# ahmetaa/fast-dnn

Measured on AMD Instinct MI355X. Metric: acoustic frames/sec (whole node), 7x2048->8000 nnet, higher is better.
Workload: dtype int8 (u8 activations x s8 weights -> int32; fp32 layer 0 and soft-max)

## Files before the change

fast-dnn_amd/api.py:

```python
from __future__ import annotations

import ctypes as C
import os
import subprocess
from typing import Optional, Sequence

import numpy as np

_HERE = os.path.dirname(os.path.abspath(__file__))
LIB_PATH = os.environ.get("FDNN_LIB") or os.path.join(_HERE, "lib", "libfast-dnn.so")
CSRC = os.path.join(_HERE, "csrc")

FDNN_OK, FDNN_E_ARG, FDNN_E_IO, FDNN_E_FORMAT, FDNN_E_DEVICE, FDNN_E_NOMEM, FDNN_E_STATE = 0, -1, -2, -3, -4, -5, -6


class FdnnError(RuntimeError):
    def __init__(self, code: int, msg: str):
        super().__init__(f"fdnn error {code}: {msg}")
        self.code = code


def build(verbose: bool = False) -> str:
    jobs = str(max(1, min(8, os.cpu_count() or 1)))
    subprocess.check_call(["make", "-C", CSRC, "-j", jobs, "all"] + ([] if verbose else ["-s"]))
# ... 23 lines not shown
    "fdnn_model_set_l0_fma": (C.c_int, [C.c_void_p, C.c_int]),
    "fdnn_debug_set_l0_kernel": (C.c_int, [C.c_void_p, C.c_int]),
    "fdnn_debug_set_chain": (C.c_int, [C.c_int, C.c_int]),
    "fdnn_model_chain_faults": (C.c_int, [C.c_void_p, C.POINTER(C.c_ulonglong)]),
    "fdnn_debug_set_pp": (C.c_int, [C.c_int, C.c_int]),
    "fdnn_debug_set_ppo": (C.c_int, [C.c_int]),
    "fdnn_debug_launch_name_count": (C.c_int, []),
    "fdnn_debug_launch_name": (C.c_char_p, [C.c_int, C.POINTER(C.c_int)]),
    "fdnn_debug_launch_record": (C.c_int, [C.c_int]),
    "fdnn_debug_launch_reset": (C.c_int, []),
    "fdnn_debug_launch_counts": (C.c_int, [C.POINTER(C.c_ulonglong), C.c_int]),
    "fdnn_debug_raise_fuse_fault": (C.c_int, [C.c_void_p, C.c_int]),
    "fdnn_device_shared": (C.c_int, [C.c_int]),
    "fdnn_debug_set_fuse": (C.c_int, [C.c_int]),
    "fdnn_debug_set_l0_list_cap": (C.c_int, [C.c_void_p, C.c_int]),
    "fdnn_debug_chain_clocks": (C.c_int, [C.c_void_p, C.POINTER(C.c_longlong), C.c_int]),
    "fdnn_calculate": (C.c_int, [C.c_void_p, _c_f32p, C.c_int, C.c_int, C.c_int, _c_f32p]),
    "fdnn_calculate_device": (C.c_int, [C.c_void_p, C.c_void_p, C.c_int, C.c_void_p, C.c_void_p]),
    "fdnn_calculate_lazy": (C.c_int, [C.c_void_p, _c_f32p, C.c_int, C.c_int, _c_i8p, _c_f32p]),
    "fdnn_calculate_lazy_bits": (C.c_int, [C.c_void_p, _c_f32p, C.c_int, C.c_int, C.POINTER(C.c_uint64), _c_f32p]),
    "fdnn_calculate_lazy_bits_device": (C.c_int, [C.c_void_p, C.c_void_p, C.c_int, C.c_void_p, C.c_void_p, C.c_void_p]),
    "fdnn_ctx_create": (C.c_int, [C.c_void_p, C.c_int, C.c_int, C.POINTER(C.c_void_p)]),
    "fdnn_ctx_free": (None, [C.c_void_p]),
    "fdnn_ctx_frame_count": (C.c_int, [C.c_void_p]),
    "fdnn_ctx_output_dim": (C.c_int, [C.c_void_p]),
    "fdnn_ctx_forward_hidden": (C.c_int, [C.c_void_p, _c_f32p]),
    "fdnn_ctx_forward_hidden_device": (C.c_int, [C.c_void_p, C.c_void_p, C.c_void_p]),
    "fdnn_ctx_lazy_output": (C.c_int, [C.c_void_p, C.c_int, _c_i8p, _c_f32p]),
    "fdnn_ctx_lazy_output_batch": (C.c_int, [C.c_void_p, C.c_int, C.c_int, _c_i8p, _c_f32p]),
    "fdnn_ctx_lazy_output_batch_device": (C.c_int, [C.c_void_p, C.c_int, C.c_int, C.c_void_p, C.c_void_p, C.c_void_p]),
# ... 123 lines not shown
def device_count() -> int:
    return int(lib().fdnn_device_count())


def device_shared(device: int = 0) -> bool:
    r = int(lib().fdnn_device_shared(int(device)))
    if r < 0:
        _check(r)
    return r == 1


def set_fuse(mode: int) -> None:
    _check(lib().fdnn_debug_set_fuse(int(mode)))


def set_chain(mode: int, min_frames: int = 0) -> None:
    _check(lib().fdnn_debug_set_chain(int(mode), int(min_frames)))


def set_pp(mode: int, min_frames: int = 0) -> None:
    _check(lib().fdnn_debug_set_pp(int(mode), int(min_frames)))


def set_ppo(mode: int) -> None:
    _check(lib().fdnn_debug_set_ppo(int(mode)))


LAUNCH_ABLATION, LAUNCH_LOAD_TIME = 1, 2


# ... 621 lines not shown
```

fast-dnn_amd/csrc/fdnn_debug.cpp:

```cpp
#include <hip/hip_runtime.h>

#include <algorithm>
#include <atomic>
#include <cstring>
#include <mutex>
#include <string>
#include <vector>

#include "fdnn_internal.hpp"

using namespace fdnn;

struct fdnn_host_model {
  fdnn::HostModel hm;
};

namespace fdnn {
const LaunchNameInfo kLaunchNames[kLaunchNameCount] = {
#define FDNN_X(id, name, flags) {name, flags},
    FDNN_LAUNCH_NAMES(FDNN_X)
#undef FDNN_X
#define FDNN_G(out, shape, branch, name, abl) {name, abl},
        FDNN_GEMM_LAUNCH_NAMES(FDNN_G)
#undef FDNN_G
// ... 40 lines not shown
    fdnn::lazy_expand_rows_from(out, comp, count, size_t(O), size_t(stride), bits);
  }
  lazy_expand_force_scalar(false);
  return FDNN_OK;
}

int fdnn_debug_set_l0_list_cap(fdnn_model *m, int cap) {
  if (!m || cap < 0) return fail(FDNN_E_ARG, "bad argument");
  std::lock_guard<std::mutex> lk(m->mu);
  for (fdnn_ctx *c : m->pool) destroy_ctx(c);
  m->pool.clear();
  m->l0_list_cap = cap;
  return FDNN_OK;
}

int fdnn_debug_set_pp(int mode, int min_frames) {
  if (mode < -1 || mode > 1) return fail(FDNN_E_ARG, "pp mode must be -1, 0 or 1");
  fdnn::qpp_set_mode(mode, min_frames);
  return FDNN_OK;
}

int fdnn_debug_raise_fuse_fault(fdnn_model *m, int value) {
  if (!m) return fail(FDNN_E_ARG, "null model");
  if (!m->h_fuse_fault) return fail(FDNN_E_STATE, "this model has no fault word");
  __atomic_store_n(m->h_fuse_fault, value ? 1ull : 0ull, __ATOMIC_RELAXED);
  if (!value) m->fuse_fault_said = false;
  return FDNN_OK;
}

int fdnn_debug_set_ppo(int mode) {
// ... 172 lines not shown
  const BlobHeader &h = m->hm.hdr;
  fdnn_ctx *c = nullptr;
  int rc = make_ctx(m, n, &c);
  if (rc) return rc;
  const size_t outs = size_t(n) * h.hidden;
  unsigned long long before[2] = {0, 0}, after[2] = {0, 0};
  hipError_t e = hipSuccess;
  if (screen) {
    e = hipMalloc(reinterpret_cast<void **>(&c->d_l0_dbg_t), outs * sizeof(float));
    if (e == hipSuccess) e = hipMalloc(reinterpret_cast<void **>(&c->d_l0_dbg_dd), outs * sizeof(float));
    if (e == hipSuccess) e = hipMemset(c->d_l0_dbg_t, 0xff, outs * sizeof(float));
    if (e == hipSuccess) e = hipMemset(c->d_l0_dbg_dd, 0xff, outs * sizeof(float));
    if (e == hipSuccess) e = hipDeviceSynchronize();
  }
  if (e == hipSuccess) e = hipMemcpy(before, m->d_l0_stats, sizeof(before), hipMemcpyDeviceToHost);
  if (e == hipSuccess) e = hipMemcpyAsync(c->d_x, x, sizeof(float) * size_t(n) * h.in_dim, hipMemcpyHostToDevice, c->stream);
  if (e == hipSuccess) {
    const int kernel_before = m->l0_kernel;
    if (screen && m->l0_kernel == 0) m->l0_kernel = 4;
    run_layer0(c, c->d_x, c->stream, nullptr);
    m->l0_kernel = kernel_before;
    e = hipGetLastError();
  }
  std::vector<int8_t> tmp(size_t(n) * size_t(c->act_ld));
  if (e == hipSuccess) e = hipMemcpyAsync(tmp.data(), c->d_act[0], tmp.size(), hipMemcpyDeviceToHost, c->stream);
  if (e == hipSuccess && screen) e = hipMemcpyAsync(t_out, c->d_l0_dbg_t, outs * sizeof(float), hipMemcpyDeviceToHost, c->stream);
  if (e == hipSuccess && screen) e = hipMemcpyAsync(dd_out, c->d_l0_dbg_dd, outs * sizeof(float), hipMemcpyDeviceToHost, c->stream);
  if (e == hipSuccess) e = hipStreamSynchronize(c->stream);
  if (e == hipSuccess) e = hipMemcpy(after, m->d_l0_stats, sizeof(after), hipMemcpyDeviceToHost);
  const size_t act_ld = size_t(c->act_ld);
// ... 158 lines not shown
```

fast-dnn_amd/csrc/fdnn_kernels.hpp:

```cpp
#pragma once
#include <hip/hip_runtime.h>

#include <cstdint>
#include <vector>

#include "fdnn_note.hpp"

#ifdef FDNN_ABLATION
#include <cstdlib>
#define FDNN_TUNE_ENV(name) std::getenv(name)
#else
#define FDNN_TUNE_ENV(name) static_cast<const char *>(nullptr)
#if (defined(FDNN_GEMM_DEBUG) && FDNN_GEMM_DEBUG) || (defined(FDNN_L0S_DEBUG) && FDNN_L0S_DEBUG) || (defined(FDNN_L0_DEBUG) && FDNN_L0_DEBUG) || \
    (defined(FDNN_CHAIN_CLK) && FDNN_CHAIN_CLK) || defined(FDNN_L0S_CLK) || defined(FDNN_GEMM_PAD)
#error "ablation / clock builds need -DFDNN_ABLATION (tools/build_variant.sh)"
#endif
#endif

namespace fdnn {

constexpr int kMaxFrameTile = 320;
constexpr int kPartialNodes = 64;

struct L0Params {
// ... 23 lines not shown
  float *xstat;
  const int8_t *wd;
  const float *wstat;
  uint2 *glist;
  uint32_t *glist_count;
  int glist_cap;
  const uint32_t *luthalf;
  float *dbg_t;
  float *dbg_dd;
};
constexpr int kL0ScreenCap = 4096;
void launch_l0(const L0Params &p, hipStream_t s);
bool l0_split_ok(int D, int H);
size_t l0_split_plane_bytes(int D, int rows_ld);
void launch_l0_split(const L0Params &p, hipStream_t s);
void l0_split_build_weights(const float *w, const float *wnorm, const uint8_t *lut2, int H, int D, int h_ld, std::vector<int8_t> *planes,
                            std::vector<float> *stat, std::vector<uint32_t> *half);
int l0_chunk_rows(int D);
int l0_chain_node_tile();
void launch_l0_weight_image(const float *w, float *wt, int H, int D, int j_pad, int h_ld, hipStream_t s);

int qgemm_frame_tile(int rows_pad, int n);
int qgemm_node_tile(int rows_pad, int n, bool output);
int qgemm_debug_flags();

struct QGemmParams {
  const int8_t *w;
  const int8_t *a;
  const float *bias;
  const int32_t *wsum;
// ... 99 lines not shown
```

fast-dnn_amd/csrc/fdnn_l0s.hip:

```cpp
#include <atomic>
#include <cmath>
#include <cstdlib>
#include <limits>
#include <type_traits>
#include <vector>

#include "fdnn_device.hpp"
#include "fdnn_kernels.hpp"

namespace fdnn {

namespace {

#ifndef FDNN_L0S_DEBUG
#define FDNN_L0S_DEBUG 0
#endif
constexpr float kU = 5.9604645e-8f;
constexpr int kSplitW = 32;

[[maybe_unused]] __device__ __forceinline__ bool split_tile_of_block(int node_tiles, int frame_tiles, int &bx, int &by) {
  const int b = blockIdx.x, xcd = b & 7, slot = b >> 3;
  bx = slot % node_tiles;
  by = xcd + 8 * (slot / node_tiles);
  return by < frame_tiles;
}

constexpr int kDigFrames = 8;
__global__ __launch_bounds__(256) void l0_digits_kernel(L0Params p, int KC, int J, int JP) {
  extern __shared__ __attribute__((aligned(16))) float dig_smem[];
  const int D = p.D, ld = D + 1;
  float *xs = dig_smem;
  float *cf_s = dig_smem + kDigFrames * ld;
  const int tid = threadIdx.x, f0 = blockIdx.x * kDigFrames;
  if (blockIdx.x == 0 && tid < 2) p.glist_count[tid] = 0u;
  const int quads = D >> 2;
  {
    float4 raw[4], sh[4], sc[4];
    int rowq[4];
#pragma unroll
    for (int it = 0; it < 4; ++it) {
// ... 91 lines not shown
      char *base = reinterpret_cast<char *>(p.xd) + ((static_cast<size_t>(kc) * 3 + pl) * blocks + (f >> 5)) * 1024 + hh * 512 + (f & 31) * 16;
      *reinterpret_cast<uint4 *>(base) = make_uint4(d[0], d[1], d[2], d[3]);
    }
  }
}

constexpr int kSTF = 128, kSStages = 3;
template <int WN>
struct SplitCfg {
  static constexpr int TN = 64 * WN, NW = 4 * WN, THREADS = 64 * NW;
  static constexpr int PIECES = 12 + 6 * WN;
  static constexpr int STAGE = PIECES * 1024;
  static constexpr int RING = STAGE * kSStages;
  static constexpr int HALF_OFF = RING;
  static constexpr int STAT_OFF = RING + 11 * 1024;
  static constexpr int LDS = STAT_OFF + 3 * 1024;
  static constexpr int TS = TN + 16;
  static constexpr int PPW = (PIECES + NW - 1) / NW;
  static_assert(kSTF * TS + 16 + 2 * kL0ScreenCap <= RING, "epilogue tile and flag list must fit in the dead ring");
};
static_assert(4 * kLut2Size <= 11 * 1024, "half-step table area");

template <int WN, bool DBG = false>
__global__ __launch_bounds__(256 * WN, 3 - WN) void l0_split_kernel(L0Params p, int KC, int CPC) {
#if defined(__HIP_DEVICE_COMPILE__)
  using Cfg = SplitCfg<WN>;
  constexpr int kSTN = Cfg::TN, kSStage = Cfg::STAGE, kSTS = Cfg::TS, kSHalfOff = Cfg::HALF_OFF, kSStatOff = Cfg::STAT_OFF, NW = Cfg::NW;
  extern __shared__ __attribute__((aligned(16))) char smem[];
  const int tid = threadIdx.x, lane = tid & 63;
  const int wave = __builtin_amdgcn_readfirstlane(tid >> 6);
  const int l32 = lane & 31, h = lane >> 5;
  const int wf = wave & 3, wn = wave >> 2;
  const int node_tiles = p.h_ld / kSTN, frame_tiles = (p.n_rows + kSTF - 1) / kSTF;
  int bx, by;
  if (!split_tile_of_block(node_tiles, frame_tiles, bx, by)) return;
  const int f0 = by * kSTF, n0 = bx * kSTN;
  const int xblocks = p.n_ld >> 5, wblocks = p.h_ld >> 5;
#ifdef FDNN_L0S_CLK
  long long tc[12];
  tc[0] = __builtin_readcyclecounter();
#define L0S_TS(i) tc[i] = __builtin_readcyclecounter()
#else
#define L0S_TS(i)
#endif

  {
    const __amdgpu_buffer_rsrc_t rsrc_half =
        __builtin_amdgcn_make_buffer_rsrc(const_cast<uint32_t *>(p.luthalf), 0, (4 * kLut2Size + 15) & ~15, 0x00020000);
#pragma unroll
    for (int i = 0; i < 14; ++i) {
      if (i % NW != wave) continue;
      if (i < 11) {
        __builtin_amdgcn_raw_ptr_buffer_load_lds(rsrc_half, FDNN_LDS_PTR(smem + kSHalfOff + i * 1024), 16, lane * 16, i * 1024, 0, 0);
      } else {
        const int q = i - 11;
        const __amdgpu_buffer_rsrc_t rsrc_st =
            __builtin_amdgcn_make_buffer_rsrc(const_cast<float *>(p.xstat + static_cast<size_t>(q) * p.n_ld + f0), 0, kSTF * 4, 0x00020000);
        __builtin_amdgcn_raw_ptr_buffer_load_lds(rsrc_st, FDNN_LDS_PTR(smem + kSStatOff + q * 1024), 16, lane * 16, 0, 0, 0);
      }
    }
  }
  const __amdgpu_buffer_rsrc_t rsrc_x =
      __builtin_amdgcn_make_buffer_rsrc(const_cast<int8_t *>(p.xd), 0, static_cast<unsigned>(KC) * 3u * static_cast<unsigned>(xblocks) * 1024u, 0x00020000);
  const __amdgpu_buffer_rsrc_t rsrc_w = __builtin_amdgcn_make_buffer_rsrc(
      const_cast<int8_t *>(p.wd), 0, static_cast<unsigned>(KC) * 3u * static_cast<unsigned>(wblocks) * 1024u, 0x00020000);
  const int voff = lane * 16;
  const int my_pieces = (Cfg::PIECES - wave + NW - 1) / NW;
  auto stage_piece = [&](int kc, int buf, int t) {
    char *base = smem + buf * kSStage;
    const int i = wave + NW * t;
    if (i >= Cfg::PIECES) return;
    if (i < 12) {
      const int pl = i >> 2, q = i & 3;
      __builtin_amdgcn_raw_ptr_buffer_load_lds(rsrc_x, FDNN_LDS_PTR(base + i * 1024), 16, voff, ((kc * 3 + pl) * xblocks + (f0 >> 5) + q) * 1024, 0, 0);
    } else {
      const int j = i - 12, pl = j / (2 * WN), q = j % (2 * WN);
      __builtin_amdgcn_raw_ptr_buffer_load_lds(rsrc_w, FDNN_LDS_PTR(base + i * 1024), 16, voff, ((kc * 3 + pl) * wblocks + (n0 >> 5) + q) * 1024, 0, 0);
    }
  };
  auto stage = [&](int kc, int buf) {
#pragma unroll
    for (int t = 0; t < Cfg::PPW; ++t) stage_piece(kc, buf, t);
  };
  auto wait_stages = [&](int stages) {
    if (stages == 0) {
      asm volatile("s_waitcnt vmcnt(0) lgkmcnt(0)" ::: "memory");
    } else if (Cfg::PIECES % NW == 0) {
      if (stages == 1)
        asm volatile("s_waitcnt vmcnt(%0) lgkmcnt(0)" ::"n"(Cfg::PPW) : "memory");
      else
        asm volatile("s_waitcnt vmcnt(%0) lgkmcnt(0)" ::"n"(2 * Cfg::PPW) : "memory");
    } else if (my_pieces == Cfg::PPW) {
      if (stages == 1)
        asm volatile("s_waitcnt vmcnt(%0) lgkmcnt(0)" ::"n"(Cfg::PPW) : "memory");
      else
        asm volatile("s_waitcnt vmcnt(%0) lgkmcnt(0)" ::"n"(2 * Cfg::PPW) : "memory");
    } else {
      if (stages == 1)
        asm volatile("s_waitcnt vmcnt(%0) lgkmcnt(0)" ::"n"(Cfg::PPW - 1) : "memory");
      else
        asm volatile("s_waitcnt vmcnt(%0) lgkmcnt(0)" ::"n"(2 * (Cfg::PPW - 1)) : "memory");
    }
  };
  stage(0, 0);
  stage(1, 1);
  stage(2, 2);
  asm volatile("" ::: "memory");

  constexpr int kP0Off = 0x40000000;
  v16i P0[2], P1[2], P2[2];
  uint32_t A[2][16];
#pragma unroll
  for (int s = 0; s < 2; ++s)
#pragma unroll
    for (int r = 0; r < 16; ++r) {
      P0[s][r] = kP0Off; P1[s][r] = 0; P2[s][r] = 0;
      A[s][r] = 0u;
    }
  auto chain_end = [&](int s) {
#pragma unroll
    for (int r = 0; r < 16; ++r) {
      P1[s][r] += P0[s][r] << 8;
      P0[s][r] = kP0Off;
    }
  };
  v4i xa[2][3], wb[2][3][2];
  auto load_plane = [&](int buf, int set, int pl) {
    const char *sb = smem + buf * kSStage;
    xa[set][pl] = *reinterpret_cast<const v4i *>(sb + (pl * 4 + wf) * 1024 + lane * 16);
#pragma unroll
    for (int s = 0; s < 2; ++s) wb[set][pl][s] = *reinterpret_cast<const v4i *>(sb + 12288 + (pl * 2 * WN + wn * 2 + s) * 1024 + lane * 16);
  };
  auto load_frags = [&](int buf, int set) {
// ... 31 lines not shown
    P1[s] = __builtin_amdgcn_mfma_i32_32x32x32_i8(xa[set][1], wb[set][0][s], P1[s], 0, 0, 0);
    FDNN_L0S_FENCE;
    sample_part(ss, 9, 12, on);
    x3();
    FDNN_L0S_FENCE;
    P2[s] = __builtin_amdgcn_mfma_i32_32x32x32_i8(xa[set][1], wb[set][1][s], P2[s], 0, 0, 0);
    FDNN_L0S_FENCE;
    sample_part(ss, 12, 16, on);
    x4();
    FDNN_L0S_FENCE;
    P2[s] = __builtin_amdgcn_mfma_i32_32x32x32_i8(xa[set][2], wb[set][0][s], P2[s], 0, 0, 0);
    FDNN_L0S_FENCE;
  };
  auto nothing = [] {};

  wait_stages(2);
  __builtin_amdgcn_s_barrier();
  asm volatile("" ::: "memory");
  load_frags(0, 0);
  L0S_TS(1);
  auto chunk = [&](int kc, auto set_c, auto first_c, bool chain_start) {
    constexpr int set = decltype(set_c)::value;
    constexpr bool first = decltype(first_c)::value;
    if (chain_start) chain_end(0);
    mfma_group(set, 0, 1, !first, nothing, nothing, nothing, nothing, nothing);
    const bool more = kc + 1 < KC, refill = kc + 3 < KC && !(FDNN_L0S_DEBUG & 8);
    if (more) {
      wait_stages(kc + 2 < KC ? 1 : 0);
      if (!(FDNN_L0S_DEBUG & 16)) __builtin_amdgcn_s_barrier();
      asm volatile("" ::: "memory");
    }
    if (chain_start) chain_end(1);
    const int nb = (kc + 1) % 3;
    mfma_group(
        set, 1, 0, true, [&] { if (more && !(FDNN_L0S_DEBUG & 32)) load_plane(nb, set ^ 1, 0); if (refill) stage_piece(kc + 3, kc % 3, 0); },
        [&] { if (more && !(FDNN_L0S_DEBUG & 32)) load_plane(nb, set ^ 1, 1); if (refill) stage_piece(kc + 3, kc % 3, 1); },
        [&] { if (more && !(FDNN_L0S_DEBUG & 32)) load_plane(nb, set ^ 1, 2); if (refill) stage_piece(kc + 3, kc % 3, 2); },
        [&] { if (refill && Cfg::PPW > 3) stage_piece(kc + 3, kc % 3, 3); }, [&] { if (refill && Cfg::PPW > 4) stage_piece(kc + 3, kc % 3, 4); });
  };
  using C0 = std::integral_constant<int, 0>;
  using C1 = std::integral_constant<int, 1>;
  chunk(0, C0{}, std::true_type{}, false);
  chunk(1, C1{}, std::false_type{}, false);
  for (int kc = 2, in_chain = 2; kc < KC; kc += 2, in_chain += 2) {
    const bool chain_start = in_chain == CPC;
    if (chain_start) in_chain = 0;
    chunk(kc, C0{}, std::false_type{}, chain_start);
    chunk(kc + 1, C1{}, std::false_type{}, false);
  }
  sample_part(1, 0, 16, true);
  chain_end(0);
  chain_end(1);
  L0S_TS(2);

  __syncthreads();
  const char *half_b = smem + kSHalfOff + 4 * kLut2Half;
  const float *rf_s = reinterpret_cast<const float *>(smem + kSStatOff);
  const float *xn_s = rf_s + 256, *af_s = rf_s + 512;
  uint8_t *tile = reinterpret_cast<uint8_t *>(smem);
  uint32_t *scr_n = reinterpret_cast<uint32_t *>(tile + kSTF * kSTS);
  uint16_t *scr_l = reinterpret_cast<uint16_t *>(tile + kSTF * kSTS + 16);
  if (tid == 0) *scr_n = 0;
  const float fD = static_cast<float>(p.D);
  const float c2 = 1.001f * (0.5f * fD * fD + 2.0f * fD) * kU;
  const float kA = 1.00001f * 256.0f * 1.002f * kU * (kSplitW + 3);
  const float kS = 100.001f * 1.002f * kU * (kSplitW / 2 + 2 + c2);
  float bias100[2], rn100[2], kSw2[2], bn2[2], eb2[2];
  bool node_in[2];
#pragma unroll
  for (int s = 0; s < 2; ++s) {
    const int node = n0 + wn * 64 + s * 32 + l32;
    node_in[s] = node < p.H;
    const float b = node_in[s] ? p.bias[node] : 0.0f;
    bias100[s] = 100.0f * b;
    rn100[s] = 100.0f * (node_in[s] ? p.wstat[node] : 0.0f);
    kSw2[s] = kS * (node_in[s] ? p.wstat[p.h_ld + node] : 0.0f);
    bn2[s] = 1.00001f * (node_in[s] ? p.wstat[2 * p.h_ld + node] : 0.0f);
    eb2[s] = 100.001f * 10.0f * kU * fabsf(b);
  }
  uint32_t valid = 0;
#pragma unroll
  for (int r = 0; r < 16; ++r) {
    const bool row_in = f0 + wf * 32 + 8 * (r >> 2) + 4 * h + (r & 3) < p.n;
    valid |= (row_in && node_in[0] ? 1u : 0u) << r;
    valid |= (row_in && node_in[1] ? 1u : 0u) << (16 + r);
  }
  float tt[2][16], sg[2][16];
  uint32_t ent[2][16];
#pragma unroll
  for (int r = 0; r < 16; ++r) {
    const float rf = rf_s[wf * 32 + 8 * (r >> 2) + 4 * h + (r & 3)];
#pragma unroll
    for (int s = 0; s < 2; ++s) {
      const float v = fmaf(static_cast<float>(P2[s][r]), 0.00390625f, static_cast<float>(P1[s][r]));
      sg[s][r] = rf * rn100[s];
      tt[s][r] = fmaf(v, sg[s][r], bias100[s]);
      const int u = max(-kLut2Half, min(kLut2Half, static_cast<int>(tt[s][r] + tt[s][r])));
      ent[s][r] = *reinterpret_cast<const uint32_t *>(half_b + 4 * u);
    }
  }
  uint32_t scr_mask = 0;
#pragma unroll
  for (int r = 0; r < 16; ++r) {
    const int row = wf * 32 + 8 * (r >> 2) + 4 * h + (r & 3);
    const float xn = xn_s[row], af = af_s[row];
#pragma unroll
    for (int s = 0; s < 2; ++s) {
      const float t = tt[s][r], sig = sg[s][r];
      tile[row * kSTS + wn * 64 + s * 32 + l32] = static_cast<uint8_t>(ent[s][r]);
      if (!(FDNN_L0S_DEBUG & 4)) {
        const float e = __builtin_amdgcn_fractf(t) - 0.5f;
        const float Dd = fmaf(fabsf(t), 12.0f * kU, fmaf(sig, fmaf(kA, static_cast<float>(A[s][r]), af + bn2[s]), fmaf(kSw2[s], xn, eb2[s]))) + 1e-30f;
        const float gate = __builtin_bit_cast(float, ent[s][r] & 0xffff0000u);
        const float m = fmaxf(fmaxf(fabsf(e), gate), fabsf(t) - 641.0f);
        const bool flag = !(m > Dd) | !(fabsf(t) < 1.0e9f);
        scr_mask |= flag ? (1u << (16 * s + r)) : 0u;
        if (DBG && ((valid >> (16 * s + r)) & 1u)) {
          const size_t o = static_cast<size_t>(f0 + row) * p.H + (n0 + wn * 64 + s * 32 + l32);
          p.dbg_t[o] = t;
          p.dbg_dd[o] = Dd;
        }
      }
    }
  }
  scr_mask &= valid;
  L0S_TS(3);
  __syncthreads();
  L0S_TS(4);
  {
    const int mine = __popc(scr_mask);
    int incl = mine;
#pragma unroll
    for (int off = 1; off < 64; off <<= 1) {
      const int v = __shfl_up(incl, off);
      if (lane >= off) incl += v;
    }
    const int wave_total = __shfl(incl, 63);
    if (wave_total) {
      uint32_t base = 0;
      if (lane == 63) base = atomicAdd(scr_n, static_cast<uint32_t>(wave_total));
      base = __shfl(base, 63);
      uint32_t at = base + static_cast<uint32_t>(incl - mine);
      uint32_t m = scr_mask;
      while (m) {
        const int i = __ffs(m) - 1;
        m &= m - 1;
        const int r = i & 15, sb2 = i >> 4;
        const int row = wf * 32 + 8 * (r >> 2) + 4 * h + (r & 3), col = wn * 64 + sb2 * 32 + l32;
        if (at < static_cast<uint32_t>(kL0ScreenCap)) scr_l[at] = static_cast<uint16_t>(row * kSTN + col);
        ++at;
      }
    }
  }
#pragma unroll
  for (int q = 0; q < kSTF * (kSTN / 16) / Cfg::THREADS; ++q) {
    const int item = tid + q * Cfg::THREADS, row = item / (kSTN / 16), c16 = (item % (kSTN / 16)) * 16;
    const int f = f0 + row;
    if (f < p.n_rows && n0 + c16 < p.H)
      *reinterpret_cast<uint4 *>(p.act_out + static_cast<size_t>(f) * p.act_ld + n0 + c16) = *reinterpret_cast<const uint4 *>(tile + row * kSTS + c16);
  }
  __syncthreads();
  {
    const uint32_t cnt = *scr_n;
    uint32_t *gbase_s = scr_n + 1;
    if (tid == 0) {
      uint32_t gb = 0xffffffffu, fill_from = 0xffffffffu;
      if (cnt != 0 && cnt <= static_cast<uint32_t>(kL0ScreenCap)) {
        gb = atomicAdd(p.glist_count, cnt);
        if (gb + cnt > static_cast<uint32_t>(p.glist_cap)) {
          fill_from = gb;
          gb = 0xffffffffu;
        }
      }
      if (cnt != 0 && gb == 0xffffffffu) {
        p.scr_count[by * (p.h_ld / 128) + (n0 >> 7)] = cnt;
        atomicAdd(p.glist_count + 1, 1u);
      }
      *gbase_s = gb;
      gbase_s[1] = fill_from;
    }
    __syncthreads();
    const uint32_t gb = *gbase_s, fill_from = gbase_s[1];
    if (fill_from < static_cast<uint32_t>(p.glist_cap))
      for (uint32_t i = fill_from + tid; i < static_cast<uint32_t>(p.glist_cap); i += Cfg::THREADS) p.glist[i] = make_uint2(0xffffffffu, 0xffffffffu);
    if (gb != 0xffffffffu)
      for (uint32_t i = tid; i < cnt; i += Cfg::THREADS) {
        const uint32_t e = scr_l[i];
        p.glist[gb + i] = make_uint2(static_cast<uint32_t>(f0) + e / kSTN, static_cast<uint32_t>(n0) + e % kSTN);
      }
  }
#ifdef FDNN_L0S_CLK
  L0S_TS(5);
  if (p.scr_stats && lane == 0 && wave == 0 && (blockIdx.x == 0 || blockIdx.x == gridDim.x / 2 + 3)) {
    unsigned long long *o = p.scr_stats + 4 + (blockIdx.x == 0 ? 0 : 12);
    for (int i = 0; i < 6; ++i) o[i] = static_cast<unsigned long long>(tc[i] - tc[0]);
  }
#endif
#endif
}

}

bool l0_split_ok(int D, int H) { return D >= 64 && D <= 496 && (D & 3) == 0 && (H & 15) == 0; }
int l0_split_chain_pad(int D) { return (D / 4 + 63) / 64 * 64; }
int l0_split_chunks(int D) { return 4 * l0_split_chain_pad(D) / 32; }
size_t l0_split_plane_bytes(int D, int rows_ld) { return static_cast<size_t>(l0_split_chunks(D)) * 3 * static_cast<size_t>(rows_ld / 32) * 1024; }
size_t l0_split_half_bytes() { return (4 * size_t(kLut2Size) + 15) & ~size_t(15); }

void l0_split_build_weights(const float *w, const float *wnorm, const uint8_t *lut2, int H, int D, int h_ld, std::vector<int8_t> *planes,
                            std::vector<float> *stat, std::vector<uint32_t> *half) {
  const int J = D / 4, JP = l0_split_chain_pad(D);
  planes->assign(l0_split_plane_bytes(D, h_ld), 0);
// ... 37 lines not shown
      for (int pl = 0; pl < 3; ++pl)
        (*planes)[((static_cast<size_t>(kc) * 3 + pl) * blocks + (n >> 5)) * 1024 + hh * 512 + (n & 31) * 16 + e] = static_cast<int8_t>(digit[pl]);
    }
    const double b_n = (u * (kSplitW + 3) * m * 0.502 * n1W / 65536.0 + std::ldexp(0.5 * n1W, -32) + std::ldexp(128.0 * (n1W2 + n1W3), -24) +
                        std::ldexp(128.0 * n1W3, -32)) * 1.002;
    auto up = [](double v) {
      float f = static_cast<float>(v);
      if (static_cast<double>(f) < v) f = std::nextafter(f, std::numeric_limits<float>::infinity());
      return f;
    };
    (*stat)[n] = 256.0f / cn;
    (*stat)[static_cast<size_t>(h_ld) + n] = wnorm[n];
    (*stat)[static_cast<size_t>(2) * h_ld + n] = degenerate ? std::numeric_limits<float>::infinity() : up(256.0 * b_n);
  }
}

void launch_l0_split(const L0Params &p, hipStream_t s) {
  const int KC = l0_split_chunks(p.D), J = p.D / 4, JP = l0_split_chain_pad(p.D);
  static std::atomic<unsigned long long> attr_set{0};
  int dev = 0;
  (void)hipGetDevice(&dev);
  const unsigned long long dev_bit = 1ull << (dev & 63);
  const int dig_lds = (kDigFrames * (p.D + 1) + kDigFrames) * 4;
  static const int wn_forced = [] {
    const char *e = FDNN_TUNE_ENV("FDNN_L0S_WN");
    return e ? std::atoi(e) : 0;
  }();
  const int tiles128 = ((p.n_rows + kSTF - 1) / kSTF) * (p.h_ld / 128);
  const int wn_cfg = wn_forced == 1 || wn_forced == 2 ? wn_forced : (tiles128 <= 128 ? 1 : 2);
  if (!(attr_set.load(std::memory_order_acquire) & dev_bit)) {
    (void)hipFuncSetAttribute(reinterpret_cast<const void *>(l0_split_kernel<1>), hipFuncAttributeMaxDynamicSharedMemorySize, SplitCfg<1>::LDS);
    (void)hipFuncSetAttribute(reinterpret_cast<const void *>(l0_split_kernel<2>), hipFuncAttributeMaxDynamicSharedMemorySize, SplitCfg<2>::LDS);
    attr_set.fetch_or(dev_bit, std::memory_order_release);
  }
  const int frame_tiles = (p.n_rows + kSTF - 1) / kSTF;
  const int dig_rows = frame_tiles * kSTF;
  note_launch(kLn_l0_digits);
  hipLaunchKernelGGL(l0_digits_kernel, dim3(dig_rows / kDigFrames), dim3(256), dig_lds, s, p, KC, J, JP);
  if (p.dbg_t != nullptr && p.dbg_dd != nullptr) {
    (void)hipFuncSetAttribute(reinterpret_cast<const void *>(l0_split_kernel<2, true>), hipFuncAttributeMaxDynamicSharedMemorySize, SplitCfg<2>::LDS);
    note_launch(kLn_l0_split_n128_probe);
    hipLaunchKernelGGL((l0_split_kernel<2, true>), dim3(static_cast<unsigned>(p.h_ld / 128) * ((frame_tiles + 7) / 8) * 8), dim3(512), SplitCfg<2>::LDS, s, p, KC, JP / 32);
    return;
  }
  note_launch(wn_cfg == 2 ? kLn_l0_split_n128 : kLn_l0_split_n64);
  if (wn_cfg == 2)
    hipLaunchKernelGGL(l0_split_kernel<2>, dim3(static_cast<unsigned>(p.h_ld / 128) * ((frame_tiles + 7) / 8) * 8), dim3(512), SplitCfg<2>::LDS, s, p, KC, JP / 32);
  else
    hipLaunchKernelGGL(l0_split_kernel<1>, dim3(static_cast<unsigned>(p.h_ld / 64) * ((frame_tiles + 7) / 8) * 8), dim3(256), SplitCfg<1>::LDS, s, p, KC, JP / 32);
}

}
```

include/fdnn.h:

```cpp
#ifndef FDNN_H
#define FDNN_H

#include <stddef.h>
#include <stdint.h>

#ifdef __cplusplus
extern "C" {
#endif

#define FDNN_API __attribute__((visibility("default")))

typedef enum fdnn_status {
  FDNN_OK = 0,
  FDNN_E_ARG = -1,
  FDNN_E_IO = -2,
  FDNN_E_FORMAT = -3,
  FDNN_E_DEVICE = -4,
  FDNN_E_NOMEM = -5,
  FDNN_E_STATE = -6
} fdnn_status;

typedef struct fdnn_model fdnn_model;
typedef struct fdnn_ctx fdnn_ctx;

// ... 88 lines not shown

FDNN_API int fdnn_debug_production_acc_out(fdnn_model *m, const float *x, int n, int stride, const int8_t *masks, int32_t *acc,
                                           float *probs);

FDNN_API int fdnn_debug_frame_chunks(int n, int *chunks, int cap);
FDNN_API int fdnn_debug_frame_chunks_for(int n, int chained, int *chunks, int cap);

FDNN_API int fdnn_debug_set_l0_kernel(fdnn_model *m, int kind);

FDNN_API int fdnn_debug_set_fuse(int mode);

FDNN_API int fdnn_debug_lazy_expand(float *out, const float *comp, int count, int O, int stride, const uint64_t *bits, int mode);

FDNN_API int fdnn_debug_set_l0_list_cap(fdnn_model *m, int cap);

FDNN_API int fdnn_debug_set_chain(int mode, int min_frames);

FDNN_API int fdnn_debug_set_pp(int mode, int min_frames);

FDNN_API int fdnn_debug_set_ppo(int mode);

FDNN_API int fdnn_debug_launch_name_count(void);
FDNN_API const char *fdnn_debug_launch_name(int index, int *flags);
FDNN_API int fdnn_debug_launch_record(int on);
FDNN_API int fdnn_debug_launch_reset(void);
FDNN_API int fdnn_debug_launch_counts(unsigned long long *out, int cap);

FDNN_API int fdnn_debug_raise_fuse_fault(fdnn_model *m, int value);

FDNN_API int fdnn_debug_chain_clocks(fdnn_ctx *c, long long *out, int cap_tasks);
// ... 39 lines not shown
```

Before: 16.26 million.

## Make layer-0 split kernel persistent with cross-tile prefetch and cached node constants

Converts the layer-0 split GEMM kernel into a persistent kernel with a grid capped by CU count times occupancy; each workgroup loops over several tiles in an XCD-aware schedule. For the 128-wide config it prefetches the next tile's first three stages and frame stats into a separate LDS region before running the current epilogue, overlapping loads with epilogue work. Per-node bias and weight-stat constants are cached in LDS and recomputed only when the node tile changes, and kernel arguments are read through the kernarg pointer. This costs more LDS per workgroup and a more complex loop, with a debug knob to cap the grid.

Result: faster. 16.45 million, median of 6 (+1.1%).

```diff
diff --git a/fast-dnn_amd/api.py b/fast-dnn_amd/api.py
--- a/fast-dnn_amd/api.py
+++ b/fast-dnn_amd/api.py
@@ -61,6 +61,7 @@
     "fdnn_device_shared": (C.c_int, [C.c_int]),
     "fdnn_debug_set_fuse": (C.c_int, [C.c_int]),
     "fdnn_debug_set_l0_list_cap": (C.c_int, [C.c_void_p, C.c_int]),
+    "fdnn_debug_set_l0_split_grid": (C.c_int, [C.c_int]),
     "fdnn_debug_chain_clocks": (C.c_int, [C.c_void_p, C.POINTER(C.c_longlong), C.c_int]),
     "fdnn_calculate": (C.c_int, [C.c_void_p, _c_f32p, C.c_int, C.c_int, C.c_int, _c_f32p]),
     "fdnn_calculate_device": (C.c_int, [C.c_void_p, C.c_void_p, C.c_int, C.c_void_p, C.c_void_p]),
@@ -214,6 +215,10 @@
     _check(lib().fdnn_debug_set_fuse(int(mode)))
 
 
+def set_l0_split_grid(wgs: int) -> None:
+    _check(lib().fdnn_debug_set_l0_split_grid(int(wgs)))
+
+
 def set_chain(mode: int, min_frames: int = 0) -> None:
     _check(lib().fdnn_debug_set_chain(int(mode), int(min_frames)))
 
diff --git a/fast-dnn_amd/csrc/fdnn_debug.cpp b/fast-dnn_amd/csrc/fdnn_debug.cpp
--- a/fast-dnn_amd/csrc/fdnn_debug.cpp
+++ b/fast-dnn_amd/csrc/fdnn_debug.cpp
@@ -78,6 +78,12 @@
   return FDNN_OK;
 }
 
+int fdnn_debug_set_l0_split_grid(int wgs) {
+  if (wgs < 0) return fail(FDNN_E_ARG, "grid cap must be 0 (default) or positive");
+  fdnn::l0_split_set_grid_cap(wgs);
+  return FDNN_OK;
+}
+
 int fdnn_debug_set_pp(int mode, int min_frames) {
   if (mode < -1 || mode > 1) return fail(FDNN_E_ARG, "pp mode must be -1, 0 or 1");
   fdnn::qpp_set_mode(mode, min_frames);
@@ -280,6 +286,7 @@
     if (e == hipSuccess) e = hipDeviceSynchronize();
   }
   if (e == hipSuccess) e = hipMemcpy(before, m->d_l0_stats, sizeof(before), hipMemcpyDeviceToHost);
+  if (e == hipSuccess) e = hipMemsetAsync(c->d_act[0], 0xa5, size_t(n) * size_t(c->act_ld), c->stream);
   if (e == hipSuccess) e = hipMemcpyAsync(c->d_x, x, sizeof(float) * size_t(n) * h.in_dim, hipMemcpyHostToDevice, c->stream);
   if (e == hipSuccess) {
     const int kernel_before = m->l0_kernel;
diff --git a/fast-dnn_amd/csrc/fdnn_kernels.hpp b/fast-dnn_amd/csrc/fdnn_kernels.hpp
--- a/fast-dnn_amd/csrc/fdnn_kernels.hpp
+++ b/fast-dnn_amd/csrc/fdnn_kernels.hpp
@@ -61,6 +61,7 @@
 bool l0_split_ok(int D, int H);
 size_t l0_split_plane_bytes(int D, int rows_ld);
 void launch_l0_split(const L0Params &p, hipStream_t s);
+void l0_split_set_grid_cap(int wgs);
 void l0_split_build_weights(const float *w, const float *wnorm, const uint8_t *lut2, int H, int D, int h_ld, std::vector<int8_t> *planes,
                             std::vector<float> *stat, std::vector<uint32_t> *half);
 int l0_chunk_rows(int D);
diff --git a/fast-dnn_amd/csrc/fdnn_l0_sched.hpp b/fast-dnn_amd/csrc/fdnn_l0_sched.hpp
--- /dev/null
+++ b/fast-dnn_amd/csrc/fdnn_l0_sched.hpp
@@ -0,0 +1,27 @@
+#pragma once
+
+#if defined(__HIPCC__) || defined(__CUDACC__)
+#define FDNN_L0_SCHED_FN __host__ __device__ inline
+#else
+#define FDNN_L0_SCHED_FN inline
+#endif
+
+namespace fdnn {
+
+FDNN_L0_SCHED_FN int l0_sched_full_grid(int node_tiles, int frame_tiles) { return node_tiles * ((frame_tiles + 7) / 8) * 8; }
+
+FDNN_L0_SCHED_FN int l0_sched_grid(int node_tiles, int frame_tiles, int max_wgs) {
+  const int full = l0_sched_full_grid(node_tiles, frame_tiles);
+  const int cap = (max_wgs + 7) / 8 * 8;
+  return cap < full ? cap : full;
+}
+
+FDNN_L0_SCHED_FN bool l0_sched_tile(int grid, int node_tiles, int frame_tiles, int b, int j, int *bx, int *by) {
+  const int xcd = b & 7, slot = b >> 3, per_xcd = grid >> 3;
+  const int i = slot + j * per_xcd;
+  *bx = i % node_tiles;
+  *by = xcd + 8 * (i / node_tiles);
+  return *by < frame_tiles;
+}
+
+}
diff --git a/fast-dnn_amd/csrc/fdnn_l0s.hip b/fast-dnn_amd/csrc/fdnn_l0s.hip
--- a/fast-dnn_amd/csrc/fdnn_l0s.hip
+++ b/fast-dnn_amd/csrc/fdnn_l0s.hip
@@ -1,3 +1,4 @@
+#include <algorithm>
 #include <atomic>
 #include <cmath>
 #include <cstdlib>
@@ -7,6 +8,7 @@
 
 #include "fdnn_device.hpp"
 #include "fdnn_kernels.hpp"
+#include "fdnn_l0_sched.hpp"
 
 namespace fdnn {
 
@@ -17,13 +19,6 @@
 #endif
 constexpr float kU = 5.9604645e-8f;
 constexpr int kSplitW = 32;
-
-[[maybe_unused]] __device__ __forceinline__ bool split_tile_of_block(int node_tiles, int frame_tiles, int &bx, int &by) {
-  const int b = blockIdx.x, xcd = b & 7, slot = b >> 3;
-  bx = slot % node_tiles;
-  by = xcd + 8 * (slot / node_tiles);
-  return by < frame_tiles;
-}
 
 constexpr int kDigFrames = 8;
 __global__ __launch_bounds__(256) void l0_digits_kernel(L0Params p, int KC, int J, int JP) {
@@ -145,10 +140,15 @@
   static constexpr int RING = STAGE * kSStages;
   static constexpr int HALF_OFF = RING;
   static constexpr int STAT_OFF = RING + 11 * 1024;
-  static constexpr int LDS = STAT_OFF + 3 * 1024;
+  static constexpr int NODE_OFF = STAT_OFF + 2 * 3 * 1024;
   static constexpr int TS = TN + 16;
+  static constexpr int EPI = kSTF * TS + 16 + 2 * kL0ScreenCap;
+  static constexpr bool AHEAD = WN == 2;
+  static constexpr int EPI_OFF = AHEAD ? NODE_OFF + 5 * TN * 4 : 0;
+  static constexpr int LDS = AHEAD ? EPI_OFF + EPI : NODE_OFF + 5 * TN * 4;
   static constexpr int PPW = (PIECES + NW - 1) / NW;
-  static_assert(kSTF * TS + 16 + 2 * kL0ScreenCap <= RING, "epilogue tile and flag list must fit in the dead ring");
+  static_assert(EPI <= RING, "epilogue tile and flag list must fit in the dead ring");
+  static_assert(LDS * (3 - WN) <= 160 * 1024, "workgroups per CU");
 };
 static_assert(4 * kLut2Size <= 11 * 1024, "half-step table area");
 
@@ -160,53 +160,65 @@
   extern __shared__ __attribute__((aligned(16))) char smem[];
   const int tid = threadIdx.x, lane = tid & 63;
   const int wave = __builtin_amdgcn_readfirstlane(tid >> 6);
-  const int l32 = lane & 31, h = lane >> 5;
   const int wf = wave & 3, wn = wave >> 2;
-  const int node_tiles = p.h_ld / kSTN, frame_tiles = (p.n_rows + kSTF - 1) / kSTF;
+  typedef const __attribute__((address_space(4))) L0Params *KP;
+  KP kp = (KP)__builtin_amdgcn_kernarg_segment_ptr();
+  (void)p;
+#define L0S_LAUNDER() asm volatile("" : "+s"(kp)::"memory")
+  const int grid = static_cast<int>(gridDim.x), wg = static_cast<int>(blockIdx.x);
+  auto my_tile = [&](int j, int *tx, int *ty) { return l0_sched_tile(grid, kp->h_ld / kSTN, (kp->n_rows + kSTF - 1) / kSTF, wg, j, tx, ty); };
   int bx, by;
-  if (!split_tile_of_block(node_tiles, frame_tiles, bx, by)) return;
-  const int f0 = by * kSTF, n0 = bx * kSTN;
-  const int xblocks = p.n_ld >> 5, wblocks = p.h_ld >> 5;
+  if (!my_tile(0, &bx, &by)) return;
+  const int xblocks = kp->n_ld >> 5, wblocks = kp->h_ld >> 5;
 #ifdef FDNN_L0S_CLK
-  long long tc[12];
-  tc[0] = __builtin_readcyclecounter();
+  long long tc[6], tc_prev_end = __builtin_readcyclecounter();
+  int clk_tiles = 1;
+  {
+    int tx, ty;
+    while (my_tile(clk_tiles, &tx, &ty)) ++clk_tiles;
+  }
 #define L0S_TS(i) tc[i] = __builtin_readcyclecounter()
 #else
 #define L0S_TS(i)
 #endif
 
+  auto stage_stats = [&](int f0_t, int set) {
+#pragma unroll
+    for (int i = 11; i < 14; ++i) {
+      if (i % NW != wave) continue;
+      const int q = i - 11;
+      const __amdgpu_buffer_rsrc_t rsrc_st =
+          __builtin_amdgcn_make_buffer_rsrc(const_cast<float *>(kp->xstat + static_cast<size_t>(q) * kp->n_ld + f0_t), 0, kSTF * 4, 0x00020000);
+      __builtin_amdgcn_raw_ptr_buffer_load_lds(rsrc_st, FDNN_LDS_PTR(smem + kSStatOff + (set * 3 + q) * 1024), 16, lane * 16, 0, 0, 0);
+    }
+  };
   {
     const __amdgpu_buffer_rsrc_t rsrc_half =
-        __builtin_amdgcn_make_buffer_rsrc(const_cast<uint32_t *>(p.luthalf), 0, (4 * kLut2Size + 15) & ~15, 0x00020000);
-#pragma unroll
-    for (int i = 0; i < 14; ++i) {
+        __builtin_amdgcn_make_buffer_rsrc(const_cast<uint32_t *>(kp->luthalf), 0, (4 * kLut2Size + 15) & ~15, 0x00020000);
+#pragma unroll
+    for (int i = 0; i < 11; ++i) {
       if (i % NW != wave) continue;
-      if (i < 11) {
-        __builtin_amdgcn_raw_ptr_buffer_load_lds(rsrc_half, FDNN_LDS_PTR(smem + kSHalfOff + i * 1024), 16, lane * 16, i * 1024, 0, 0);
-      } else {
-        const int q = i - 11;
-        const __amdgpu_buffer_rsrc_t rsrc_st =
-            __builtin_amdgcn_make_buffer_rsrc(const_cast<float *>(p.xstat + static_cast<size_t>(q) * p.n_ld + f0), 0, kSTF * 4, 0x00020000);
-        __builtin_amdgcn_raw_ptr_buffer_load_lds(rsrc_st, FDNN_LDS_PTR(smem + kSStatOff + q * 1024), 16, lane * 16, 0, 0, 0);
-      }
-    }
+      __builtin_amdgcn_raw_ptr_buffer_load_lds(rsrc_half, FDNN_LDS_PTR(smem + kSHalfOff + i * 1024), 16, lane * 16, i * 1024, 0, 0);
+    }
+    stage_stats(by * kSTF, 0);
   }
   const __amdgpu_buffer_rsrc_t rsrc_x =
-      __builtin_amdgcn_make_buffer_rsrc(const_cast<int8_t *>(p.xd), 0, static_cast<unsigned>(KC) * 3u * static_cast<unsigned>(xblocks) * 1024u, 0x00020000);
+      __builtin_amdgcn_make_buffer_rsrc(const_cast<int8_t *>(kp->xd), 0, static_cast<unsigned>(KC) * 3u * static_cast<unsigned>(xblocks) * 1024u, 0x00020000);
   const __amdgpu_buffer_rsrc_t rsrc_w = __builtin_amdgcn_make_buffer_rsrc(
-      const_cast<int8_t *>(p.wd), 0, static_cast<unsigned>(KC) * 3u * static_cast<unsigned>(wblocks) * 1024u, 0x00020000);
+      const_cast<int8_t *>(kp->wd), 0, static_cast<unsigned>(KC) * 3u * static_cast<unsigned>(wblocks) * 1024u, 0x00020000);
   const int voff = lane * 16;
   const int my_pieces = (Cfg::PIECES - wave + NW - 1) / NW;
+  int sxb = by * (kSTF / 32), snb = bx * (kSTN / 32);
   auto stage_piece = [&](int kc, int buf, int t) {
     char *base = smem + buf * kSStage;
     const int i = wave + NW * t;
     if (i >= Cfg::PIECES) return;
     if (i < 12) {
       const int pl = i >> 2, q = i & 3;
-      __builtin_amdgcn_raw_ptr_buffer_load_lds(rsrc_x, FDNN_LDS_PTR(base + i * 1024), 16, voff, ((kc * 3 + pl) * xblocks + (f0 >> 5) + q) * 1024, 0, 0);
+      __builtin_amdgcn_raw_ptr_buffer_load_lds(rsrc_x, FDNN_LDS_PTR(base + i * 1024), 16, voff, ((kc * 3 + pl) * xblocks + sxb + q) * 1024, 0, 0);
     } else {
       const int j = i - 12, pl = j / (2 * WN), q = j % (2 * WN);
-      __builtin_amdgcn_raw_ptr_buffer_load_lds(rsrc_w, FDNN_LDS_PTR(base + i * 1024), 16, voff, ((kc * 3 + pl) * wblocks + (n0 >> 5) + q) * 1024, 0, 0);
+      __builtin_amdgcn_raw_ptr_buffer_load_lds(rsrc_w, FDNN_LDS_PTR(base + i * 1024), 16, voff, ((kc * 3 + pl) * wblocks + snb + q) * 1024, 0, 0);
     }
   };
   auto stage = [&](int kc, int buf) {
@@ -233,21 +245,18 @@
         asm volatile("s_waitcnt vmcnt(%0) lgkmcnt(0)" ::"n"(2 * (Cfg::PPW - 1)) : "memory");
     }
   };
-  stage(0, 0);
-  stage(1, 1);
-  stage(2, 2);
-  asm volatile("" ::: "memory");
-
   constexpr int kP0Off = 0x40000000;
   v16i P0[2], P1[2], P2[2];
   uint32_t A[2][16];
-#pragma unroll
-  for (int s = 0; s < 2; ++s)
-#pragma unroll
-    for (int r = 0; r < 16; ++r) {
-      P0[s][r] = kP0Off; P1[s][r] = 0; P2[s][r] = 0;
-      A[s][r] = 0u;
-    }
+  auto reset_acc = [&] {
+#pragma unroll
+    for (int s = 0; s < 2; ++s)
+#pragma unroll
+      for (int r = 0; r < 16; ++r) {
+        P0[s][r] = kP0Off; P1[s][r] = 0; P2[s][r] = 0;
+        A[s][r] = 0u;
+      }
+  };
   auto chain_end = [&](int s) {
 #pragma unroll
     for (int r = 0; r < 16; ++r) {
@@ -309,11 +318,6 @@
   };
   auto nothing = [] {};
 
-  wait_stages(2);
-  __builtin_amdgcn_s_barrier();
-  asm volatile("" ::: "memory");
-  load_frags(0, 0);
-  L0S_TS(1);
   auto chunk = [&](int kc, auto set_c, auto first_c, bool chain_start) {
     constexpr int set = decltype(set_c)::value;
     constexpr bool first = decltype(first_c)::value;
@@ -335,6 +339,28 @@
   };
   using C0 = std::integral_constant<int, 0>;
   using C1 = std::integral_constant<int, 1>;
+
+  constexpr float kA = 1.00001f * 256.0f * 1.002f * kU * (kSplitW + 3);
+  float *nodec = reinterpret_cast<float *>(smem + Cfg::NODE_OFF);
+  int node_bx = -1;
+  stage(0, 0);
+  stage(1, 1);
+  stage(2, 2);
+  asm volatile("" ::: "memory");
+
+  for (int t = 0;; ++t) {
+  const int f0 = by * kSTF, n0 = bx * kSTN, set_t = t & 1;
+  L0S_LAUNDER();
+  L0S_TS(0);
+  reset_acc();
+  if (t == 0)
+    wait_stages(2);
+  else
+    wait_stages(0);
+  __builtin_amdgcn_s_barrier();
+  asm volatile("" ::: "memory");
+  load_frags(0, 0);
+  L0S_TS(1);
   chunk(0, C0{}, std::true_type{}, false);
   chunk(1, C1{}, std::false_type{}, false);
   for (int kc = 2, in_chain = 2; kc < KC; kc += 2, in_chain += 2) {
@@ -346,41 +372,78 @@
   sample_part(1, 0, 16, true);
   chain_end(0);
   chain_end(1);
+#pragma unroll
+  for (int set = 0; set < 2; ++set)
+#pragma unroll
+    for (int pl = 0; pl < 3; ++pl) {
+      asm volatile("" : "=v"(xa[set][pl]));
+      asm volatile("" : "=v"(wb[set][pl][0]));
+      asm volatile("" : "=v"(wb[set][pl][1]));
+    }
   L0S_TS(2);
 
   __syncthreads();
+  int nbx, nby;
+  const bool has_next = my_tile(t + 1, &nbx, &nby);
+  auto stage_next = [&] {
+    sxb = nby * (kSTF / 32);
+    snb = nbx * (kSTN / 32);
+    stage(0, 0);
+    stage(1, 1);
+    stage(2, 2);
+    stage_stats(nby * kSTF, set_t ^ 1);
+    asm volatile("" ::: "memory");
+  };
+  if (Cfg::AHEAD && has_next) stage_next();
+  L0S_LAUNDER();
+  int tid_l = tid;
+  asm volatile("" : "+v"(tid_l));
+  {
+  const int tid = tid_l, lane = tid & 63, l32 = lane & 31, h = lane >> 5;
   const char *half_b = smem + kSHalfOff + 4 * kLut2Half;
-  const float *rf_s = reinterpret_cast<const float *>(smem + kSStatOff);
+  const float *rf_s = reinterpret_cast<const float *>(smem + kSStatOff + set_t * 3 * 1024);
   const float *xn_s = rf_s + 256, *af_s = rf_s + 512;
-  uint8_t *tile = reinterpret_cast<uint8_t *>(smem);
+  uint8_t *tile = reinterpret_cast<uint8_t *>(smem + Cfg::EPI_OFF);
   uint32_t *scr_n = reinterpret_cast<uint32_t *>(tile + kSTF * kSTS);
   uint16_t *scr_l = reinterpret_cast<uint16_t *>(tile + kSTF * kSTS + 16);
   if (tid == 0) *scr_n = 0;
-  const float fD = static_cast<float>(p.D);
-  const float c2 = 1.001f * (0.5f * fD * fD + 2.0f * fD) * kU;
-  const float kA = 1.00001f * 256.0f * 1.002f * kU * (kSplitW + 3);
-  const float kS = 100.001f * 1.002f * kU * (kSplitW / 2 + 2 + c2);
+  if (bx != node_bx) {
+    if (tid < kSTN) {
+      const float fD = static_cast<float>(kp->D);
+      const float c2 = 1.001f * (0.5f * fD * fD + 2.0f * fD) * kU;
+      const float kS = 100.001f * 1.002f * kU * (kSplitW / 2 + 2 + c2);
+      const int node = n0 + tid;
+      const bool in = node < kp->H;
+      const float b = in ? kp->bias[node] : 0.0f;
+      nodec[tid] = 100.0f * b;
+      nodec[kSTN + tid] = 100.0f * (in ? kp->wstat[node] : 0.0f);
+      nodec[2 * kSTN + tid] = kS * (in ? kp->wstat[kp->h_ld + node] : 0.0f);
+      nodec[3 * kSTN + tid] = 1.00001f * (in ? kp->wstat[2 * kp->h_ld + node] : 0.0f);
+      nodec[4 * kSTN + tid] = 100.001f * 10.0f * kU * fabsf(b);
+    }
+    node_bx = bx;
+    __syncthreads();
+  }
   float bias100[2], rn100[2], kSw2[2], bn2[2], eb2[2];
   bool node_in[2];
 #pragma unroll
   for (int s = 0; s < 2; ++s) {
-    const int node = n0 + wn * 64 + s * 32 + l32;
-    node_in[s] = node < p.H;
-    const float b = node_in[s] ? p.bias[node] : 0.0f;
-    bias100[s] = 100.0f * b;
-    rn100[s] = 100.0f * (node_in[s] ? p.wstat[node] : 0.0f);
-    kSw2[s] = kS * (node_in[s] ? p.wstat[p.h_ld + node] : 0.0f);
-    bn2[s] = 1.00001f * (node_in[s] ? p.wstat[2 * p.h_ld + node] : 0.0f);
-    eb2[s] = 100.001f * 10.0f * kU * fabsf(b);
+    const int col = wn * 64 + s * 32 + l32;
+    node_in[s] = n0 + col < kp->H;
+    bias100[s] = nodec[col];
+    rn100[s] = nodec[kSTN + col];
+    kSw2[s] = nodec[2 * kSTN + col];
+    bn2[s] = nodec[3 * kSTN + col];
+    eb2[s] = nodec[4 * kSTN + col];
   }
   uint32_t valid = 0;
 #pragma unroll
   for (int r = 0; r < 16; ++r) {
-    const bool row_in = f0 + wf * 32 + 8 * (r >> 2) + 4 * h + (r & 3) < p.n;
+    const bool row_in = f0 + wf * 32 + 8 * (r >> 2) + 4 * h + (r & 3) < kp->n;
     valid |= (row_in && node_in[0] ? 1u : 0u) << r;
     valid |= (row_in && node_in[1] ? 1u : 0u) << (16 + r);
   }
-  float tt[2][16], sg[2][16];
+  float tt[2][16];
   uint32_t ent[2][16];
 #pragma unroll
   for (int r = 0; r < 16; ++r) {
@@ -388,8 +451,7 @@
 #pragma unroll
     for (int s = 0; s < 2; ++s) {
       const float v = fmaf(static_cast<float>(P2[s][r]), 0.00390625f, static_cast<float>(P1[s][r]));
-      sg[s][r] = rf * rn100[s];
-      tt[s][r] = fmaf(v, sg[s][r], bias100[s]);
+      tt[s][r] = fmaf(v, rf * rn100[s], bias100[s]);
       const int u = max(-kLut2Half, min(kLut2Half, static_cast<int>(tt[s][r] + tt[s][r])));
       ent[s][r] = *reinterpret_cast<const uint32_t *>(half_b + 4 * u);
     }
@@ -398,10 +460,10 @@
 #pragma unroll
   for (int r = 0; r < 16; ++r) {
     const int row = wf * 32 + 8 * (r >> 2) + 4 * h + (r & 3);
-    const float xn = xn_s[row], af = af_s[row];
+    const float xn = xn_s[row], af = af_s[row], rf = rf_s[row];
 #pragma unroll
     for (int s = 0; s < 2; ++s) {
-      const float t = tt[s][r], sig = sg[s][r];
+      const float t = tt[s][r], sig = rf * rn100[s];
       tile[row * kSTS + wn * 64 + s * 32 + l32] = static_cast<uint8_t>(ent[s][r]);
       if (!(FDNN_L0S_DEBUG & 4)) {
         const float e = __builtin_amdgcn_fractf(t) - 0.5f;
@@ -411,9 +473,9 @@
         const bool flag = !(m > Dd) | !(fabsf(t) < 1.0e9f);
         scr_mask |= flag ? (1u << (16 * s + r)) : 0u;
         if (DBG && ((valid >> (16 * s + r)) & 1u)) {
-          const size_t o = static_cast<size_t>(f0 + row) * p.H + (n0 + wn * 64 + s * 32 + l32);
-          p.dbg_t[o] = t;
-          p.dbg_dd[o] = Dd;
+          const size_t o = static_cast<size_t>(f0 + row) * kp->H + (n0 + wn * 64 + s * 32 + l32);
+          kp->dbg_t[o] = t;
+          kp->dbg_dd[o] = Dd;
         }
       }
     }
@@ -430,11 +492,11 @@
       const int v = __shfl_up(incl, off);
       if (lane >= off) incl += v;
     }
-    const int wave_total = __shfl(incl, 63);
+    const int wave_total = __builtin_amdgcn_readlane(incl, 63);
     if (wave_total) {
       uint32_t base = 0;
       if (lane == 63) base = atomicAdd(scr_n, static_cast<uint32_t>(wave_total));
-      base = __shfl(base, 63);
+      base = static_cast<uint32_t>(__builtin_amdgcn_readlane(static_cast<int>(base), 63));
       uint32_t at = base + static_cast<uint32_t>(incl - mine);
       uint32_t m = scr_mask;
       while (m) {
@@ -451,8 +513,8 @@
   for (int q = 0; q < kSTF * (kSTN / 16) / Cfg::THREADS; ++q) {
     const int item = tid + q * Cfg::THREADS, row = item / (kSTN / 16), c16 = (item % (kSTN / 16)) * 16;
     const int f = f0 + row;
-    if (f < p.n_rows && n0 + c16 < p.H)
-      *reinterpret_cast<uint4 *>(p.act_out + static_cast<size_t>(f) * p.act_ld + n0 + c16) = *reinterpret_cast<const uint4 *>(tile + row * kSTS + c16);
+    if (f < kp->n_rows && n0 + c16 < kp->H)
+      *reinterpret_cast<uint4 *>(kp->act_out + static_cast<size_t>(f) * kp->act_ld + n0 + c16) = *reinterpret_cast<const uint4 *>(tile + row * kSTS + c16);
   }
   __syncthreads();
   {
@@ -461,36 +523,52 @@
     if (tid == 0) {
       uint32_t gb = 0xffffffffu, fill_from = 0xffffffffu;
       if (cnt != 0 && cnt <= static_cast<uint32_t>(kL0ScreenCap)) {
-        gb = atomicAdd(p.glist_count, cnt);
-        if (gb + cnt > static_cast<uint32_t>(p.glist_cap)) {
+        gb = atomicAdd(kp->glist_count, cnt);
+        if (gb + cnt > static_cast<uint32_t>(kp->glist_cap)) {
           fill_from = gb;
           gb = 0xffffffffu;
         }
       }
       if (cnt != 0 && gb == 0xffffffffu) {
-        p.scr_count[by * (p.h_ld / 128) + (n0 >> 7)] = cnt;
-        atomicAdd(p.glist_count + 1, 1u);
+        kp->scr_count[by * (kp->h_ld / 128) + (n0 >> 7)] = cnt;
+        atomicAdd(kp->glist_count + 1, 1u);
       }
       *gbase_s = gb;
       gbase_s[1] = fill_from;
     }
     __syncthreads();
     const uint32_t gb = *gbase_s, fill_from = gbase_s[1];
-    if (fill_from < static_cast<uint32_t>(p.glist_cap))
-      for (uint32_t i = fill_from + tid; i < static_cast<uint32_t>(p.glist_cap); i += Cfg::THREADS) p.glist[i] = make_uint2(0xffffffffu, 0xffffffffu);
+    if (fill_from < static_cast<uint32_t>(kp->glist_cap))
+      for (uint32_t i = fill_from + tid; i < static_cast<uint32_t>(kp->glist_cap); i += Cfg::THREADS) kp->glist[i] = make_uint2(0xffffffffu, 0xffffffffu);
     if (gb != 0xffffffffu)
       for (uint32_t i = tid; i < cnt; i += Cfg::THREADS) {
         const uint32_t e = scr_l[i];
-        p.glist[gb + i] = make_uint2(static_cast<uint32_t>(f0) + e / kSTN, static_cast<uint32_t>(n0) + e % kSTN);
-      }
+        kp->glist[gb + i] = make_uint2(static_cast<uint32_t>(f0) + e / kSTN, static_cast<uint32_t>(n0) + e % kSTN);
+      }
+  }
   }
 #ifdef FDNN_L0S_CLK
   L0S_TS(5);
-  if (p.scr_stats && lane == 0 && wave == 0 && (blockIdx.x == 0 || blockIdx.x == gridDim.x / 2 + 3)) {
-    unsigned long long *o = p.scr_stats + 4 + (blockIdx.x == 0 ? 0 : 12);
-    for (int i = 0; i < 6; ++i) o[i] = static_cast<unsigned long long>(tc[i] - tc[0]);
-  }
+  if (kp->scr_stats && lane == 0 && wave == 0 && (wg == 0 || wg == grid / 2 + 3)) {
+    unsigned long long *o = kp->scr_stats + 4 + (wg == 0 ? 0 : 12);
+    for (int k = 0; k < 3; ++k) {
+      if (t != (k == 0 ? 0 : k == 1 ? clk_tiles / 2 : clk_tiles - 1)) continue;
+      o[4 * k] = static_cast<unsigned long long>(tc[1] - tc_prev_end);
+      o[4 * k + 1] = static_cast<unsigned long long>(tc[2] - tc[1]);
+      o[4 * k + 2] = static_cast<unsigned long long>(tc[5] - tc[2]);
+      o[4 * k + 3] = static_cast<unsigned long long>(tc[4] - tc[2]);
+    }
+  }
+  tc_prev_end = tc[5];
 #endif
+  if (!has_next) break;
+  if (!Cfg::AHEAD) {
+    __syncthreads();
+    stage_next();
+  }
+  bx = nbx;
+  by = nby;
+  }
 #endif
 }
 
@@ -558,6 +636,9 @@
     (*stat)[static_cast<size_t>(2) * h_ld + n] = degenerate ? std::numeric_limits<float>::infinity() : up(256.0 * b_n);
   }
 }
+
+static std::atomic<int> g_split_grid_cap{0};
+void l0_split_set_grid_cap(int wgs) { g_split_grid_cap.store(wgs > 0 ? wgs : 0, std::memory_order_relaxed); }
 
 void launch_l0_split(const L0Params &p, hipStream_t s) {
   const int KC = l0_split_chunks(p.D), J = p.D / 4, JP = l0_split_chain_pad(p.D);
@@ -581,17 +662,28 @@
   const int dig_rows = frame_tiles * kSTF;
   note_launch(kLn_l0_digits);
   hipLaunchKernelGGL(l0_digits_kernel, dim3(dig_rows / kDigFrames), dim3(256), dig_lds, s, p, KC, J, JP);
+  static std::atomic<int> cu_of_dev[64];
+  int n_cu = cu_of_dev[dev & 63].load(std::memory_order_relaxed);
+  if (n_cu == 0) {
+    if (hipDeviceGetAttribute(&n_cu, hipDeviceAttributeMultiprocessorCount, dev) != hipSuccess || n_cu <= 0) n_cu = 256;
+    cu_of_dev[dev & 63].store(n_cu, std::memory_order_relaxed);
+  }
+  const int cap = g_split_grid_cap.load(std::memory_order_relaxed);
+  auto grid_of = [&](int wn) {
+    const int g = l0_sched_grid(p.h_ld / (64 * wn), frame_tiles, n_cu * (3 - wn));
+    return dim3(static_cast<unsigned>(cap > 0 ? std::min(g, (cap + 7) / 8 * 8) : g));
+  };
   if (p.dbg_t != nullptr && p.dbg_dd != nullptr) {
     (void)hipFuncSetAttribute(reinterpret_cast<const void *>(l0_split_kernel<2, true>), hipFuncAttributeMaxDynamicSharedMemorySize, SplitCfg<2>::LDS);
     note_launch(kLn_l0_split_n128_probe);
-    hipLaunchKernelGGL((l0_split_kernel<2, true>), dim3(static_cast<unsigned>(p.h_ld / 128) * ((frame_tiles + 7) / 8) * 8), dim3(512), SplitCfg<2>::LDS, s, p, KC, JP / 32);
+    hipLaunchKernelGGL((l0_split_kernel<2, true>), grid_of(2), dim3(512), SplitCfg<2>::LDS, s, p, KC, JP / 32);
     return;
   }
   note_launch(wn_cfg == 2 ? kLn_l0_split_n128 : kLn_l0_split_n64);
   if (wn_cfg == 2)
-    hipLaunchKernelGGL(l0_split_kernel<2>, dim3(static_cast<unsigned>(p.h_ld / 128) * ((frame_tiles + 7) / 8) * 8), dim3(512), SplitCfg<2>::LDS, s, p, KC, JP / 32);
+    hipLaunchKernelGGL(l0_split_kernel<2>, grid_of(2), dim3(512), SplitCfg<2>::LDS, s, p, KC, JP / 32);
   else
-    hipLaunchKernelGGL(l0_split_kernel<1>, dim3(static_cast<unsigned>(p.h_ld / 64) * ((frame_tiles + 7) / 8) * 8), dim3(256), SplitCfg<1>::LDS, s, p, KC, JP / 32);
+    hipLaunchKernelGGL(l0_split_kernel<1>, grid_of(1), dim3(256), SplitCfg<1>::LDS, s, p, KC, JP / 32);
 }
 
 }
diff --git a/include/fdnn.h b/include/fdnn.h
--- a/include/fdnn.h
+++ b/include/fdnn.h
@@ -126,6 +126,8 @@
 
 FDNN_API int fdnn_debug_set_l0_list_cap(fdnn_model *m, int cap);
 
+FDNN_API int fdnn_debug_set_l0_split_grid(int wgs);
+
 FDNN_API int fdnn_debug_set_chain(int mode, int min_frames);
 
 FDNN_API int fdnn_debug_set_pp(int mode, int min_frames);
```
